# sk4161/EgoScaler

Measured on AMD Instinct MI355X. Metric: clips/sec/GPU (8-frame 224^2, 16-token text) fwd+bwd, higher is better.
Workload: dtype bf16

## Files before the change

egoscaler_amd/_lib.py:

```python
import ctypes
import os

import torch

_HERE = os.path.dirname(os.path.abspath(__file__))
LIB_PATH = os.path.join(_HERE, "lib", "libegomi.so")
_lib = None

c_p = ctypes.c_void_p
c_i = ctypes.c_int
c_d = ctypes.c_double
c_f = ctypes.c_float
c_sz = ctypes.c_size_t
c_i64 = ctypes.c_int64


class EgomiError(RuntimeError):
    pass


def lib():
    global _lib
    if _lib is None:
        if not os.path.exists(LIB_PATH):
            raise EgomiError(f"{LIB_PATH} not found: build it with `python -m egoscaler_amd.build` "
                             "(the product path has no CPU fallback)")
        _lib = ctypes.CDLL(LIB_PATH)
        _lib.egomi_strerror.restype = ctypes.c_char_p
        _lib.egomi_strerror.argtypes = [c_i]
        _lib.egomi_last_launch_error.restype = ctypes.c_char_p
        _lib.egomi_unproject_workspace_bytes.restype = c_sz
        _lib.egomi_unproject_workspace_bytes.argtypes = [c_i] * 4
    return _lib


def check(rc: int, what: str):
    if rc != 0:
        msg = lib().egomi_strerror(rc).decode()
        if rc == -3:
            msg += ": " + lib().egomi_last_launch_error().decode()
        raise EgomiError(f"{what}: egomi error {rc} ({msg})")


_SYNC_DEBUG = os.environ.get("EGOMI_SYNC_DEBUG")


def call(name: str, *args):
    fn = getattr(lib(), name)
    if not _SYNC_DEBUG:
        check(fn(*args), name)
        return
    import traceback
    import torch
    try:
        check(fn(*args), name)
        if not torch.cuda.is_current_stream_capturing():
            torch.cuda.synchronize()
    except BaseException as e:
        with open(_SYNC_DEBUG, "a") as f:
            f.write(f"=== {name} raised {type(e).__name__}: {str(e)[:200]}\n")
            f.write("".join(traceback.format_stack(limit=14)))
            f.write(f"args: {[getattr(a, 'value', a) for a in args]}\n")
        raise
```

egoscaler_amd/csrc/attention.hip:

```cpp
#include "common.h"
#include <math.h>
#include <type_traits>

#define AT_HD 128
__device__ __forceinline__ float fast_exp2(float x) { return __builtin_amdgcn_exp2f(x); }
typedef __attribute__((ext_vector_type(4))) __bf16 bf16x4_t;
typedef __attribute__((address_space(3))) bf16x4_t lds_bf16x4;

struct AttnArgs {
    const bf16_t* q; const bf16_t* k; const bf16_t* v; bf16_t* o; float* lse;
    const bf16_t* dout; float* delta; bf16_t* dq; bf16_t* dk; bf16_t* dv;
    const uint8_t* key_mask;
    int B, H, S;
    long long ld_qkv, ld_o, ld_dqkv;
    float scale;
    int causal;
    const float* rope_cos; const float* rope_sin;
};

__device__ __forceinline__ int sw_off(int row, int ch) {
    return 256 * row + 16 * (ch ^ (((row & 3) << 2) | ((row >> 2) & 3)));
}
__device__ __forceinline__ int rowmap(int reg, int half) {
    return (reg & 3) + 8 * (reg >> 2) + 4 * half;
}
__device__ __forceinline__ uint32_t visible_bits(uint32_t km32, int half, int key0, int qi, int causal) {
    uint32_t t = km32 >> (4 * half);
    if (causal) {
        const int lim = qi - key0 - 4 * half;
        const uint32_t cb = lim < 0 ? 0u : (lim >= 31 ? 0xFFFFFFFFu : ((2u << lim) - 1u));
        t &= cb;
    }
    return t;
}
__device__ __forceinline__ bf16x8 lds_row8(const char* tile, int row, int ch) {
    return *reinterpret_cast<const bf16x8*>(tile + sw_off(row, ch));
}
__device__ __forceinline__ bf16x8 lds_tr8(const char* tile, int r0, int col0, int lane) {
    const int half = lane >> 5, q = (lane >> 2) & 3, p = lane & 3;
    const int col = col0 + 16 * ((lane >> 4) & 1) + 4 * p;
    const int ch = col >> 3, within = (col & 7) * 2;
    const int ra = r0 + 4 * half + q;
    const bf16x4_t lo = __builtin_amdgcn_ds_read_tr16_b64_v4bf16((lds_bf16x4*)(tile + sw_off(ra, ch) + within));
    const bf16x4_t hi = __builtin_amdgcn_ds_read_tr16_b64_v4bf16((lds_bf16x4*)(tile + sw_off(ra + 8, ch) + within));
    bf16x8 r;
    r[0] = lo[0]; r[1] = lo[1]; r[2] = lo[2]; r[3] = lo[3];
    r[4] = hi[0]; r[5] = hi[1]; r[6] = hi[2]; r[7] = hi[3];
    return r;
}
__device__ __forceinline__ bf16x8 pack8(const float* v) {
// ... 1650 lines not shown
            vis &= hi < 0 ? 0u : (hi >= 31 ? 0xFFFFFFFFu : ((2u << hi) - 1u));
#pragma unroll
            for (int r = 0; r < 16; ++r) pv[r] = (vis >> rowmap(r, 0)) & 1u ? pv[r] : 0.f;
        }
#pragma unroll
        for (int g = 0; g < 4; ++g) {
            const f32x4 d4 = *reinterpret_cast<const f32x4*>(sD + 8 * g + 4 * half);
#pragma unroll
            for (int e = 0; e < 4; ++e) ds[4 * g + e] = pv[4 * g + e] * (dp[4 * g + e] - d4[e]);
        }
#pragma unroll
        for (int s2 = 0; s2 < 2; ++s2) {
            const bf16x8 pb = pack8(&pv[8 * s2]);
            const bf16x8 db = pack8(&ds[8 * s2]);
#pragma unroll
            for (int dt = 0; dt < HD / 32; ++dt) {
                dv[dt] = __builtin_amdgcn_mfma_f32_32x32x16_bf16(lds_tr8_t<HD>(sDO, 16 * s2, 32 * dt, lane), pb, dv[dt], 0, 0, 0);
                dk[dt] = __builtin_amdgcn_mfma_f32_32x32x16_bf16(lds_tr8_t<HD>(sQ, 16 * s2, 32 * dt, lane), db, dk[dt], 0, 0, 0);
            }
        }
        asm volatile("s_waitcnt lgkmcnt(0)" ::: "memory");
        __builtin_amdgcn_s_barrier();
    }
    asm volatile("s_waitcnt vmcnt(0)" ::: "memory");
    __builtin_amdgcn_s_barrier();
    store_rows_t<HD>(smem + wave * (HD == 128 ? AT_XBYTES : 32 * 144), dk, a.scale, a.dk + row_base * a.ld_dqkv + h * HD, a.ld_dqkv, kb0 + wave * 32, a.S, lane,
                     a.rope_cos, a.rope_sin);
    store_rows_t<HD>(smem + wave * (HD == 128 ? AT_XBYTES : 32 * 144), dv, 1.0f, a.dv + row_base * a.ld_dqkv + h * HD, a.ld_dqkv, kb0 + wave * 32, a.S, lane);
}

__device__ __forceinline__ void dma4_asm(const void* gbase, uint32_t voff, uint32_t lds_base) {
    asm volatile("s_mov_b32 m0, %2\n\ts_nop 0\n\tglobal_load_lds_dword %0, %1" :: "v"(voff), "s"(gbase), "s"(lds_base) : "memory");
}
template <bool MASKED>
__device__ __forceinline__ void dkdv2_tile(const char* sQ, const char* sDO, const char* sVrows, const float* sL, const float* sD, const bf16x8 (&kf)[8],
                                           f32x16 (&dk)[4], f32x16 (&dv)[4], const float sc2, const uint32_t vis, const int lane, const int half) {
    f32x16 x, dp;
#pragma unroll
    for (int r = 0; r < 16; ++r) { x[r] = 0.f; dp[r] = 0.f; }
    const int row = lane & 31;
    bf16x8 qr[2], dr[2], vr[2];
    qr[0] = lds_row8(sQ, row, half); dr[0] = lds_row8(sDO, row, half); vr[0] = lds_row8(sVrows, row, half);
    __builtin_amdgcn_sched_barrier(0);
#pragma unroll
    for (int ks = 0; ks < 8; ++ks) {
        if (ks + 1 < 8) {
            qr[(ks + 1) & 1] = lds_row8(sQ, row, 2 * (ks + 1) + half);
            dr[(ks + 1) & 1] = lds_row8(sDO, row, 2 * (ks + 1) + half);
            vr[(ks + 1) & 1] = lds_row8(sVrows, row, 2 * (ks + 1) + half);
        }
        x = __builtin_amdgcn_mfma_f32_32x32x16_bf16(qr[ks & 1], kf[ks], x, 0, 0, 0);
        dp = __builtin_amdgcn_mfma_f32_32x32x16_bf16(dr[ks & 1], vr[ks & 1], dp, 0, 0, 0);
    }
    bf16x8 dot[4], qt[4];
#pragma unroll
    for (int dt = 0; dt < 4; ++dt) dot[dt] = lds_tr8(sDO, 0, 32 * dt, lane);
    float pv[16], ds[16];
#pragma unroll
    for (int g = 0; g < 4; ++g) {
        const f32x4 l4 = *reinterpret_cast<const f32x4*>(sL + 8 * g + 4 * half);
#pragma unroll
        for (int e = 0; e < 4; ++e) pv[4 * g + e] = fast_exp2(fmaf(x[4 * g + e], sc2, -l4[e] * 1.4426950408889634f));
    }
    if (MASKED) {
#pragma unroll
        for (int r = 0; r < 16; ++r) pv[r] = (vis >> rowmap(r, 0)) & 1u ? pv[r] : 0.f;
    }
#pragma unroll
    for (int dt = 0; dt < 4; ++dt) qt[dt] = lds_tr8(sQ, 0, 32 * dt, lane);
#pragma unroll
    for (int g = 0; g < 4; ++g) {
        const f32x4 d4 = *reinterpret_cast<const f32x4*>(sD + 8 * g + 4 * half);
#pragma unroll
        for (int e = 0; e < 4; ++e) ds[4 * g + e] = pv[4 * g + e] * (dp[4 * g + e] - d4[e]);
    }
    {
        const bf16x8 pb = pack8(&pv[0]);
        const bf16x8 db = pack8(&ds[0]);
#pragma unroll
        for (int dt = 0; dt < 4; ++dt) dv[dt] = __builtin_amdgcn_mfma_f32_32x32x16_bf16(dot[dt], pb, dv[dt], 0, 0, 0);
#pragma unroll
        for (int dt = 0; dt < 4; ++dt) dot[dt] = lds_tr8(sDO, 16, 32 * dt, lane);
#pragma unroll
        for (int dt = 0; dt < 4; ++dt) dk[dt] = __builtin_amdgcn_mfma_f32_32x32x16_bf16(qt[dt], db, dk[dt], 0, 0, 0);
#pragma unroll
        for (int dt = 0; dt < 4; ++dt) qt[dt] = lds_tr8(sQ, 16, 32 * dt, lane);
    }
    {
        const bf16x8 pb = pack8(&pv[8]);
        const bf16x8 db = pack8(&ds[8]);
#pragma unroll
        for (int dt = 0; dt < 4; ++dt) dv[dt] = __builtin_amdgcn_mfma_f32_32x32x16_bf16(dot[dt], pb, dv[dt], 0, 0, 0);
#pragma unroll
        for (int dt = 0; dt < 4; ++dt) dk[dt] = __builtin_amdgcn_mfma_f32_32x32x16_bf16(qt[dt], db, dk[dt], 0, 0, 0);
    }
}

__global__ __launch_bounds__(256, 2) void attn_bwd_dkdv2_kernel(AttnArgs a) {
    extern __shared__ __attribute__((aligned(16))) char smem[];
    const int lane = threadIdx.x & 63, half = lane >> 5;
    const int wave = __builtin_amdgcn_readfirstlane(threadIdx.x >> 6);
    int rank, h, b;
    attn_block_map(a, rank, h, b);
    const int kb0 = rank * 128;
    const long long row_base = (long long)b * a.S;
    const bf16_t* Q = a.q + row_base * a.ld_qkv + h * AT_HD;
    const bf16_t* K = a.k + row_base * a.ld_qkv + h * AT_HD;
    const bf16_t* V = a.v + row_base * a.ld_qkv + h * AT_HD;
    const bf16_t* DO = a.dout + row_base * a.ld_o + h * AT_HD;
    const float* LSE = a.lse + ((long long)b * a.H + h) * a.S;
    const float* DEL = a.delta + ((long long)b * a.H + h) * a.S;
    const int kj = kb0 + wave * 32 + (lane & 31);
    const int kr = kj < a.S ? kj : a.S - 1;
    bool key_ok = kj < a.S;
    if (key_ok && a.key_mask) key_ok = a.key_mask[row_base + kj] != 0;
    const bool keys_all_ok = __all(key_ok);
    const bool wave_dead = kb0 + wave * 32 >= a.S;
    char* sVblk = smem + 2 * DKV_STAGE;
    const uint32_t lds_smem = (uint32_t)(uintptr_t)((lds_void_t*)smem);
    {
        const uint32_t base = __builtin_amdgcn_readfirstlane(lds_smem + 2 * DKV_STAGE + wave * 8 * 1024);
#pragma unroll
        for (int j = 0; j < 8; ++j) {
            const int rl = (wave * 8 + j) * 4 + (lane >> 4);
            const int ch = (lane & 15) ^ (((rl & 3) << 2) | ((rl >> 2) & 3));
            int r = kb0 + rl;
            r = r < a.S ? r : a.S - 1;
            dma16_asm(V, (uint32_t)((long long)r * a.ld_qkv + ch * 8) * 2u, base + j * 1024);
        }
    }
// ... 20 lines not shown
            const int ch = (lane & 15) ^ (((rl & 3) << 2) | ((rl >> 2) & 3));
            int r = q0 + rl;
            r = r < a.S ? r : a.S - 1;
            qo[j] = (uint32_t)((long long)r * a.ld_qkv + ch * 8) * 2u;
            dofs[j] = (uint32_t)((long long)r * a.ld_o + ch * 8) * 2u;
        }
        int qq = q0 + (lane & 31);
        qq = qq < a.S ? qq : a.S - 1;
        lo = (uint32_t)qq * 4u;
    };
    offsets_for(qt0 * 32, qoff, dooff, loff);
    const uint32_t q_stride = (uint32_t)(32 * a.ld_qkv * 2), do_stride = (uint32_t)(32 * a.ld_o * 2);
    const float* LD = (wave & 1) ? DEL : LSE;
    auto issue = [&](int stage, const uint32_t (&qo)[2], const uint32_t (&dofs)[2], const uint32_t lo) {
        const uint32_t base = __builtin_amdgcn_readfirstlane(lds_smem + stage * DKV_STAGE + wave * 2 * 1024);
#pragma unroll
        for (int j = 0; j < 2; ++j) dma16_asm(Q, qo[j], base + j * 1024);
#pragma unroll
        for (int j = 0; j < 2; ++j) dma16_asm(DO, dofs[j], base + 32 * 256 + j * 1024);
        dma4_asm(LD, lo, __builtin_amdgcn_readfirstlane(lds_smem + stage * DKV_STAGE + 2 * 32 * 256 + wave * 256));
    };
    auto issue_next = [&](int qt_next, int stage) {
        if (ragged && qt_next == nq - 1) {
            uint32_t qo[2], dofs[2], lo;
            offsets_for(qt_next * 32, qo, dofs, lo);
            issue(stage, qo, dofs, lo);
        } else {
            issue(stage, qoff, dooff, loff);
#pragma unroll
            for (int j = 0; j < 2; ++j) { qoff[j] += q_stride; dooff[j] += do_stride; }
            loff += 128u;
        }
    };
    if (qt0 < nq) issue_next(qt0, 0);
    int stg = 0;
    auto top_of_tile = [&](int qt) {
        if (qt + 1 < nq) {
            issue_next(qt + 1, stg ^ 1);
            asm volatile("s_waitcnt vmcnt(5)" ::: "memory");
        } else {
            asm volatile("s_waitcnt vmcnt(0)" ::: "memory");
        }
        asm volatile("s_waitcnt lgkmcnt(0)" ::: "memory");
        __builtin_amdgcn_s_barrier();
    };
    auto end_of_tile = [&]() {
        stg ^= 1;
        asm volatile("s_waitcnt lgkmcnt(0)" ::: "memory");
        __builtin_amdgcn_s_barrier();
    };
    const char* sVrows = sVblk + wave * 32 * 256;
    auto run = [&](auto masked_tag, int qt) {
        constexpr bool MASKED = decltype(masked_tag)::value;
        const char* st = smem + stg * DKV_STAGE;
        const float* sL = reinterpret_cast<const float*>(st + 2 * 32 * 256);
        uint32_t vis = 0u;
        if (MASKED) {
            const int q0 = qt * 32;
            const int lo = a.causal ? kj - q0 - 4 * half : 0;
            const int hi = a.S - 1 - q0 - 4 * half;
            vis = key_ok ? 0xFFFFFFFFu : 0u;
            vis &= lo <= 0 ? 0xFFFFFFFFu : (lo >= 32 ? 0u : ~((1u << lo) - 1u));
            vis &= hi < 0 ? 0u : (hi >= 31 ? 0xFFFFFFFFu : ((2u << hi) - 1u));
        }
        dkdv2_tile<MASKED>(st, st + 32 * 256, sVrows, sL, sL + 64, kf, dk, dv, sc2, vis, lane, half);
    };
    using T_ = std::integral_constant<bool, true>;
    using F_ = std::integral_constant<bool, false>;
    int qt = qt0;
    const int diag = kb0 / 32 + wave;
    const int dead_end = wave_dead ? nq : (a.causal ? (diag < nq ? diag : nq) : qt0);
    for (; qt < dead_end; ++qt) {
        top_of_tile(qt);
        end_of_tile();
    }
    if (a.causal && qt < nq && qt == diag) {
        top_of_tile(qt);
        run(T_{}, qt);
        end_of_tile();
        ++qt;
    }
    if (keys_all_ok) {
        const int int_end = a.S / 32;
        for (; qt < int_end; ++qt) {
            top_of_tile(qt);
            run(F_{}, qt);
            end_of_tile();
        }
    }
    for (; qt < nq; ++qt) {
        top_of_tile(qt);
        run(T_{}, qt);
        end_of_tile();
    }
    store_rows_via_lds(smem + wave * AT_XBYTES, dk, a.scale, a.dk + row_base * a.ld_dqkv + h * AT_HD, a.ld_dqkv, kb0 + wave * 32, a.S, lane,
                       a.rope_cos, a.rope_sin);
    store_rows_via_lds(smem + wave * AT_XBYTES, dv, 1.0f, a.dv + row_base * a.ld_dqkv + h * AT_HD, a.ld_dqkv, kb0 + wave * 32, a.S, lane);
}

static int attn_occ() {
    static int occ = -1;
    if (occ < 0) { const char* e = getenv("EGOMI_ATTN_OCC"); occ = e ? atoi(e) : 3; }
    return occ;
}
static bool occ_dq2() { return attn_occ() & 1; }

static int g_attn_fwd_form = -1;
static int attn_fwd_form() {
    if (g_attn_fwd_form < 0) { const char* e = getenv("EGOMI_ATTN_FWD"); g_attn_fwd_form = e ? atoi(e) : 4; }
    return g_attn_fwd_form;
}
extern "C" int egomi_attn_set_fwd_form(int form) {
    if (form < 1 || form > 4) return EGOMI_E_BADARG;
    g_attn_fwd_form = form;
    return EGOMI_OK;
}
static int g_attn_fwd_group = -1;
static int attn_fwd_group() {
    if (g_attn_fwd_group < 0) { const char* e = getenv("EGOMI_ATTN_GROUP"); g_attn_fwd_group = e ? atoi(e) : 0; }
    return g_attn_fwd_group;
}
extern "C" int egomi_attn_set_fwd_group(int group) {
    if (group < 0 || group > 64) return EGOMI_E_BADARG;
    g_attn_fwd_group = group;
    return EGOMI_OK;
}
static int g_attn_fwd_blocks = 0;
extern "C" int egomi_attn_set_fwd_blocks(int blocks) {
    if (blocks < 0) return EGOMI_E_BADARG;
    g_attn_fwd_blocks = blocks;
    return EGOMI_OK;
}
static int g_attn_bwd_form = -1;
static int attn_bwd_form() {
    if (g_attn_bwd_form < 0) { const char* e = getenv("EGOMI_ATTN_BWD"); g_attn_bwd_form = e ? atoi(e) : 3; }
    return g_attn_bwd_form;
}
extern "C" int egomi_attn_set_bwd_form(int form) {
    if (form < 1 || form > 3) return EGOMI_E_BADARG;
    g_attn_bwd_form = form;
    return EGOMI_OK;
}

static int attn_check(const egomi_attn_desc* d, bool fwd_only = false) {
    if (!d || !d->q || !d->k || !d->v) return EGOMI_E_BADARG;
    if (d->head_dim != AT_HD && d->head_dim != 64) return EGOMI_E_UNSUPPORTED;
    (void)fwd_only;
    if (d->B <= 0 || d->H <= 0 || d->S <= 0) return EGOMI_E_SHAPE;
    if (d->dtype != EGOMI_BF16) return EGOMI_E_UNSUPPORTED;
    if (d->ld_qkv % 8 || d->ld_qkv < d->head_dim * d->H) return EGOMI_E_SHAPE;
    if (((uintptr_t)d->q | (uintptr_t)d->k | (uintptr_t)d->v) & 15) return EGOMI_E_SHAPE;
    return EGOMI_OK;
}

static AttnArgs attn_args(const egomi_attn_desc* d) {
    AttnArgs a;
    a.q = (const bf16_t*)d->q; a.k = (const bf16_t*)d->k; a.v = (const bf16_t*)d->v; a.o = (bf16_t*)d->o; a.lse = d->lse;
    a.dout = (const bf16_t*)d->dout; a.delta = d->delta; a.dq = (bf16_t*)d->dq; a.dk = (bf16_t*)d->dk; a.dv = (bf16_t*)d->dv;
    a.key_mask = d->key_mask; a.B = d->B; a.H = d->H; a.S = d->S;
    a.ld_qkv = d->ld_qkv; a.ld_o = d->ld_o; a.ld_dqkv = d->ld_dqkv; a.scale = d->scale; a.causal = d->causal;
    a.rope_cos = d->rope_cos; a.rope_sin = d->rope_sin;
    return a;
}

extern "C" int egomi_attn_fwd(const egomi_attn_desc* d, egomi_stream_t stream) {
    const int rc = attn_check(d, true);
    if (rc) return rc;
    if (!d->o || d->ld_o % 8 || d->ld_o < d->head_dim * d->H || ((uintptr_t)d->o & 15)) return EGOMI_E_SHAPE;
    if (d->S > AT_MAXS) return EGOMI_E_UNSUPPORTED;
    AttnArgs a = attn_args(d);
    const dim3 grid((unsigned)(((d->S + 127) / 128) * d->H * d->B));
    const size_t lds = 2 * 2 * 64 * 2 * (size_t)d->head_dim + (size_t)((d->S + 63) / 64) * 64;
    int form = attn_fwd_form();
    if ((long long)d->S * d->ld_qkv * 2 >= (1ll << 32)) form = 1;
    if (d->head_dim == 128 && form == 4 && d->S > 1024) form = 3;
    if (d->head_dim == 128 && form == 4) {
        const int s32 = (d->S + 31) & ~31, nblk = (s32 + 127) / 128;
        const int n_items = nblk * d->H * d->B;
        static int cus = 0;
        if (!cus) { int dev = 0; hipDeviceProp_t pr; cus = (hipGetDevice(&dev) == hipSuccess && hipGetDeviceProperties(&pr, dev) == hipSuccess) ? pr.multiProcessorCount : 256; }
        int grid4 = n_items < 2 * cus ? n_items : 2 * cus;
        if (g_attn_fwd_blocks > 0 && g_attn_fwd_blocks < grid4) grid4 = g_attn_fwd_blocks;
        const size_t lds4 = (size_t)F3_NST * F3_STAGE + 4 * F4_STRIP + 2 * (size_t)s32;
        (void)hipFuncSetAttribute(reinterpret_cast<const void*>(attn_fwd4_kernel), hipFuncAttributeMaxDynamicSharedMemorySize, (int)lds4);
        EGOMI_LAUNCH(attn_fwd4_kernel, dim3((unsigned)grid4), dim3(256), lds4, (hipStream_t)stream, a, n_items);
        return egomi_launch_status();
    }
    if (d->head_dim == 128 && form == 3) {
        const int s32 = (d->S + 31) & ~31, nblk = (s32 + 127) / 128;
        int group = (d->H * d->B) % 8 == 0 ? attn_fwd_group() : 0;
        if (group > nblk) group = nblk;
        const int nb = group > 0 ? ((nblk + group - 1) / group) * group : nblk;
        const dim3 grid3((unsigned)(nb * d->H * d->B));
        const size_t lds3 = (size_t)F3_NST * F3_STAGE + (size_t)s32;
        (void)hipFuncSetAttribute(reinterpret_cast<const void*>(attn_fwd3_kernel), hipFuncAttributeMaxDynamicSharedMemorySize, (int)lds3);
        EGOMI_LAUNCH(attn_fwd3_kernel, grid3, dim3(256), lds3, (hipStream_t)stream, a, group);
        return egomi_launch_status();
    }
    if (d->head_dim == 128) {
        if (form == 1) {
            (void)hipFuncSetAttribute(reinterpret_cast<const void*>(attn_fwd_kernel<128>), hipFuncAttributeMaxDynamicSharedMemorySize, (int)lds);
            EGOMI_LAUNCH(attn_fwd_kernel<128>, grid, dim3(256), lds, (hipStream_t)stream, a);
        } else {
            (void)hipFuncSetAttribute(reinterpret_cast<const void*>(attn_fwd2_kernel<128>), hipFuncAttributeMaxDynamicSharedMemorySize, (int)lds);
            EGOMI_LAUNCH(attn_fwd2_kernel<128>, grid, dim3(256), lds, (hipStream_t)stream, a);
        }
    } else if (form == 1) {
        EGOMI_LAUNCH(attn_fwd_kernel<64>, grid, dim3(256), lds, (hipStream_t)stream, a);
    } else {
        EGOMI_LAUNCH(attn_fwd2_kernel<64>, grid, dim3(256), lds, (hipStream_t)stream, a);
    }
    return egomi_launch_status();
}

extern "C" int egomi_attn_bwd(const egomi_attn_desc* d, egomi_stream_t stream) {
    const int rc = attn_check(d);
    if (rc) return rc;
    if (!d->o || !d->lse || !d->dout || !d->delta || !d->dq || !d->dk || !d->dv) return EGOMI_E_BADARG;
    if (d->ld_o % 8 || d->ld_dqkv % 8 || d->ld_o < d->head_dim * d->H || d->ld_dqkv < d->head_dim * d->H) return EGOMI_E_SHAPE;
    if (((uintptr_t)d->dout & 15) || (((uintptr_t)d->dq | (uintptr_t)d->dk | (uintptr_t)d->dv) & 15) || ((uintptr_t)d->o & 15)) return EGOMI_E_SHAPE;
    if (d->S > AT_MAXS) return EGOMI_E_UNSUPPORTED;
    if ((d->rope_cos == nullptr) != (d->rope_sin == nullptr)) return EGOMI_E_BADARG;
    if (d->rope_cos && (((uintptr_t)d->rope_cos | (uintptr_t)d->rope_sin) & 15)) return EGOMI_E_SHAPE;
    AttnArgs a = attn_args(d);
    hipStream_t s = (hipStream_t)stream;
    const dim3 grid((unsigned)(((d->S + 127) / 128) * d->H * d->B));
    if (d->head_dim == 64) {
        if (d->rope_cos) return EGOMI_E_UNSUPPORTED;
        const size_t lq = 2 * 2 * 64 * 128 + (size_t)((d->S + 63) / 64) * 64, lk = 2 * (2 * 32 * 128 + 4 * 256) + 128 * 128;
        EGOMI_LAUNCH((attn_bwd_dq_kernel<2, 64>), grid, dim3(256), lq, s, a);
        EGOMI_LAUNCH((attn_bwd_dkdv_kernel<2, 64>), grid, dim3(256), lk, s, a);
        return egomi_launch_status();
    }
    const size_t lds_q = ((occ_dq2() ? 2 : 3) * 2 * 64 * 256) + (size_t)((d->S + 63) / 64) * 64;
    const int occ = attn_occ();
    const bool off32 = (long long)d->S * d->ld_qkv * 2 < (1ll << 32) && (long long)d->S * d->ld_o * 2 < (1ll << 32);
    if ((occ & 1) && attn_bwd_form() == 3 && off32) {
        const size_t lds3 = (size_t)F3_NST * F3_STAGE + (size_t)((d->S + 31) & ~31);
        (void)hipFuncSetAttribute(reinterpret_cast<const void*>(attn_bwd_dq3_kernel), hipFuncAttributeMaxDynamicSharedMemorySize, (int)lds3);
        EGOMI_LAUNCH(attn_bwd_dq3_kernel, grid, dim3(256), lds3, s, a);
    } else if ((occ & 1) && attn_bwd_form() == 2 && off32) {
        (void)hipFuncSetAttribute(reinterpret_cast<const void*>(attn_bwd_dq2_kernel), hipFuncAttributeMaxDynamicSharedMemorySize, (int)lds_q);
        EGOMI_LAUNCH(attn_bwd_dq2_kernel, grid, dim3(256), lds_q, s, a);
    } else if (occ & 1) {
        (void)hipFuncSetAttribute(reinterpret_cast<const void*>(attn_bwd_dq_kernel<2>), hipFuncAttributeMaxDynamicSharedMemorySize, (int)lds_q);
        EGOMI_LAUNCH(attn_bwd_dq_kernel<2>, grid, dim3(256), lds_q, s, a);
    } else {
        (void)hipFuncSetAttribute(reinterpret_cast<const void*>(attn_bwd_dq_kernel<1>), hipFuncAttributeMaxDynamicSharedMemorySize, (int)lds_q);
        EGOMI_LAUNCH(attn_bwd_dq_kernel<1>, grid, dim3(256), lds_q, s, a);
    }
    const size_t lds_k = (occ & 2) ? 2 * DKV_STAGE + 128 * 256 : 3 * DKV_STAGE;
    if ((occ & 2) && attn_bwd_form() >= 2 && off32) {
        (void)hipFuncSetAttribute(reinterpret_cast<const void*>(attn_bwd_dkdv2_kernel), hipFuncAttributeMaxDynamicSharedMemorySize, (int)lds_k);
        EGOMI_LAUNCH(attn_bwd_dkdv2_kernel, grid, dim3(256), lds_k, s, a);
    } else if (occ & 2) {
        (void)hipFuncSetAttribute(reinterpret_cast<const void*>(attn_bwd_dkdv_kernel<2>), hipFuncAttributeMaxDynamicSharedMemorySize, (int)lds_k);
        EGOMI_LAUNCH(attn_bwd_dkdv_kernel<2>, grid, dim3(256), lds_k, s, a);
    }
    else EGOMI_LAUNCH(attn_bwd_dkdv_kernel<1>, grid, dim3(256), lds_k, s, a);
    return egomi_launch_status();
}
```

egoscaler_amd/engine.py:

```python
import os
from typing import Dict

import torch

from . import ops
from .config import EgoDims


class Workspace:

    def __init__(self, device):
        self.device = device
        self.bufs: Dict[str, torch.Tensor] = {}

    def get(self, name, shape, dtype, zero=False):
        t = self.bufs.get(name)
        shape = tuple(int(s) for s in shape)
        if t is None or t.shape != shape or t.dtype != dtype:
            t = torch.empty(shape, dtype=dtype, device=self.device)
            self.bufs[name] = t
            if zero:
                t.zero_()
        elif zero:
            t.zero_()
# ... 617 lines not shown
            lc = ctx["layers"][l]
            gu, qkv = lc["gu"], lc["qkv"]
            self._begin_direct(l)
            dgu = ws.get("dgu", (M, 2 * Fd), T)
            wt_down = self.wT.get(p + "mlp.down_proj.weight") if self.prepared else None
            if fuse_swiglu_bwd and wt_down is not None and l in self.wguT:
                ops.mm(dx, wt_down, out=dgu, swiglu_bwd_gu=gu)
            else:
                d_act = self._dgrad(dx, p + "mlp.down_proj.weight", ws.get("d_act", (M, Fd), T))
                if self.prepared and l in self.wguT and self.gu_il:
                    ops.swiglu_il_bwd(d_act, gu, dgu)
                else:
                    ops.swiglu_bwd(d_act, gu[:, :Fd], gu[:, Fd:], dgu[:, :Fd], dgu[:, Fd:])
            self._wgrad(p + "mlp.down_proj.weight", dx, lc["act"])
            t_h2 = None
            if self.prepared and l in self.wguT:
                if defer_b:
                    d_h2, t_h2 = ops.mm(dgu, self.wguT[l], out=ws.get("d_h", (M, d), T), defer_tail=True)
                else:
                    d_h2 = ops.mm(dgu, self.wguT[l], out=ws.get("d_h", (M, d), T))
            elif self.prepared and l in self.wgu_cat:
                d_h2 = self._dgrad_w(dgu, self.wgu_cat[l], ws.get("d_h", (M, d), T))
            else:
                d_h2 = self._dgrad(dgu[:, :Fd], p + "mlp.gate_proj.weight", ws.get("d_h", (M, d), T))
                self._dgrad(dgu[:, Fd:], p + "mlp.up_proj.weight", d_h2, residual=d_h2)
            self._wgrad_stacked([p + "mlp.gate_proj.weight", p + "mlp.up_proj.weight"], dgu, lc["h2"])
            n2 = p + "post_attention_layernorm.weight"
            d_mid = ops.rmsnorm_bwd(d_h2, lc["x_mid"], w[n2], lc["rstd2"], dx_add=dx,
                                    dw=self.grad_buffer(n2) if n2 in tr else None, out=ws.get("dx_b", (M, d), T), tail=t_h2)
            d_ao = self._dgrad(d_mid, p + "self_attn.o_proj.weight", ws.get("d_ao", (M, d), T))
            self._wgrad(p + "self_attn.o_proj.weight", d_mid, lc["ao"])
            dqkv = ws.get("dqkv", (M, 3 * d), T)
            if lc["lse"] is not None:
                ops.attn_bwd(qkv, lc["ao"], lc["lse"], d_ao, dqkv, ws.get("att_delta", (B, H, S), torch.float32), B, S, H, hd, scale,
                             causal=True, key_mask=ctx["key_mask"], rope=(self.cos, self.sin))
            else:
                self._attention_bwd(qkv, lc["P"], d_ao, dqkv, B, S, H, hd, scale)
                ops.rope_(dqkv, self.cos, self.sin, M, S, 0, 2 * H, hd, 3 * d, inverse=True)
            t_h = None
            if self.prepared and l in self.wqkvT:
                if defer_b:
                    d_h, t_h = ops.mm(dqkv, self.wqkvT[l], out=ws.get("d_h", (M, d), T), defer_tail=True)
                else:
                    d_h = ops.mm(dqkv, self.wqkvT[l], out=ws.get("d_h", (M, d), T))
            elif self.prepared and l in self.wqkv and self.use_tn and T == torch.bfloat16:
                d_h = self._dgrad_w(dqkv, self.wqkv[l], ws.get("d_h", (M, d), T))
            else:
                d_h = self._dgrad(dqkv[:, :d], p + "self_attn.q_proj.weight", ws.get("d_h", (M, d), T))
                self._dgrad(dqkv[:, d:2 * d], p + "self_attn.k_proj.weight", d_h, residual=d_h)
                self._dgrad(dqkv[:, 2 * d:], p + "self_attn.v_proj.weight", d_h, residual=d_h)
            self._wgrad_stacked([p + f"self_attn.{nm}_proj.weight" for nm in "qkv"], dqkv, lc["h"])
            n1 = p + "input_layernorm.weight"
            dx = ops.rmsnorm_bwd(d_h, lc["x_in"], w[n1], lc["rstd1"], dx_add=d_mid,
                                 dw=self.grad_buffer(n1) if n1 in tr else None, out=ws.get("dx_a", (M, d), T), tail=t_h)
            self._notify_layer(l)
        Pn = pb.point_token_len
        V = lm.vocab_size
        emb_name = "model.embed_tokens.weight"
        Bc = ctx["n_clouds"]
        d_feats = ws.get("d_pp_out", (Bc * Pn, d), T) if ctx["has_points"] else None
        if d_feats is not None:
            d_feats.zero_()
        ops.embed_splice_bwd(dx.view(B, S, d), ctx["ids"], ctx["start_pos"], Pn, V,
                             self.grad_buffer(emb_name) if emb_name in tr else None, d_feats, cloud_idx=ctx["cloud_idx"])
        if ctx["has_points"]:
            acts = ctx["pp_acts"]
            nh = len(pb.projection_hidden_dim)
            g = d_feats
# ... 57 lines not shown
```

egoscaler_amd/ops.py:

```python
import ctypes
import math

import torch

from . import _lib
from ._lib import c_p, c_i, c_d, c_f, c_sz, c_i64, call

F32, BF16 = 0, 1


def dt(t: torch.dtype) -> int:
    if t == torch.float32:
        return F32
    if t == torch.bfloat16:
        return BF16
    raise TypeError(f"unsupported dtype {t}")


def P(t):
    if t is None:
        return c_p(None)
    if not t.is_cuda:
        raise _lib.EgomiError("egoscaler_amd ops need CUDA/HIP tensors (no CPU fallback)")
    return c_p(t.data_ptr())
# ... 475 lines not shown

def add(a, b, out=None):
    out = torch.empty_like(a) if out is None else out
    call("egomi_add", P(a), P(b), P(out), c_i64(a.numel()), c_i(dt(a.dtype)), S())
    return out


def colsum_(x, out):
    R, C = x.shape
    call("egomi_colsum", P(x), c_i64(R), c_i(C), c_i64(_ld(x)), P(out), c_i(dt(x.dtype)), S())
    return out


def group_max(x, BG, M, C, concat=False, out=None):
    if out is None:
        out = torch.empty((BG * M, 2 * C) if concat else (BG, C), dtype=x.dtype, device=x.device)
    call("egomi_group_max", P(x), c_i(BG), c_i(M), c_i(C), P(out), c_i(int(concat)), c_i(dt(x.dtype)), S())
    return out


def linear_smallk(x, w, b, act=0, out=None):
    R, K = x.numel() // x.shape[-1], x.shape[-1]
    N = w.shape[0]
    out = torch.empty(R, N, dtype=w.dtype, device=w.device) if out is None else out
    call("egomi_linear_smallk", P(x), c_i(dt(x.dtype)), P(w), P(b), P(out), c_i64(R), c_i(N), c_i(K), c_i(act), c_i(dt(w.dtype)), S())
    return out


class AttnDesc(ctypes.Structure):
    _fields_ = [("q", c_p), ("k", c_p), ("v", c_p), ("o", c_p), ("lse", c_p),
                ("dout", c_p), ("delta", c_p), ("dq", c_p), ("dk", c_p), ("dv", c_p), ("key_mask", c_p),
                ("B", c_i), ("H", c_i), ("S", c_i), ("head_dim", c_i),
                ("ld_qkv", c_i64), ("ld_o", c_i64), ("ld_dqkv", c_i64),
                ("scale", c_f), ("causal", c_i), ("dtype", c_i), ("rope_cos", c_p), ("rope_sin", c_p)]


def _attn_desc(qkv, B, Sq, H, hd, scale, causal, key_mask):
    d = AttnDesc()
    dm = H * hd
    d.q, d.k, d.v = qkv[:, :dm].data_ptr(), qkv[:, dm:2 * dm].data_ptr(), qkv[:, 2 * dm:].data_ptr()
    d.key_mask = key_mask.data_ptr() if key_mask is not None else None
    d.B, d.H, d.S, d.head_dim = B, H, Sq, hd
    d.ld_qkv = qkv.stride(0)
    d.scale, d.causal, d.dtype = scale, int(causal), dt(qkv.dtype)
    return d


def attn_fwd(qkv, B, Sq, H, hd, scale, out, lse, causal=True, key_mask=None):
    d = _attn_desc(qkv, B, Sq, H, hd, scale, causal, key_mask)
    d.o, d.lse, d.ld_o = out.data_ptr(), lse.data_ptr() if lse is not None else None, out.stride(0)
    call("egomi_attn_fwd", ctypes.byref(d), S())
    return out


def attn_bwd(qkv, out, lse, dout, dqkv, delta, B, Sq, H, hd, scale, causal=True, key_mask=None, rope=None):
    d = _attn_desc(qkv, B, Sq, H, hd, scale, causal, key_mask)
    if rope is not None:
        cos, sin = rope
        if cos.dtype != torch.float32 or sin.dtype != torch.float32 or cos.shape[0] < Sq or cos.shape[1] != hd // 2 \
                or not cos.is_contiguous() or not sin.is_contiguous():
            raise ValueError("attn_bwd: rope tables must be contiguous fp32 [>=S, head_dim/2]")
        d.rope_cos, d.rope_sin = cos.data_ptr(), sin.data_ptr()
    dm = H * hd
    d.o, d.lse, d.ld_o = out.data_ptr(), lse.data_ptr(), out.stride(0)
    if dout.stride(0) != out.stride(0):
        raise ValueError("attn_bwd: dout and out must share their row stride")
    d.dout, d.delta = dout.data_ptr(), delta.data_ptr()
    d.dq, d.dk, d.dv = dqkv[:, :dm].data_ptr(), dqkv[:, dm:2 * dm].data_ptr(), dqkv[:, 2 * dm:].data_ptr()
    d.ld_dqkv = dqkv.stride(0)
    call("egomi_attn_bwd", ctypes.byref(d), S())
    return dqkv
```

include/egomi.h:

```cpp
#ifndef EGOMI_H
#define EGOMI_H
#include <stddef.h>
#include <stdint.h>

#ifdef __cplusplus
extern "C" {
#endif

#define EGOMI_OK 0
#define EGOMI_E_BADARG (-1)
#define EGOMI_E_SHAPE (-2)
#define EGOMI_E_LAUNCH (-3)
#define EGOMI_E_UNSUPPORTED (-4)

#define EGOMI_F32 0
#define EGOMI_BF16 1

typedef void* egomi_stream_t;

int egomi_version(void);
const char* egomi_strerror(int code);
const char* egomi_last_launch_error(void);

size_t egomi_unproject_workspace_bytes(int B, int T, int H, int W);
// ... 25 lines not shown
    float alpha;
    int accumulate;
    int act;
    int force_generic;
    void* workspace; int64_t workspace_bytes; int split_k;
    int ws_tickets_zeroed;
    int epilogue; void* C2; int64_t ldc2;
} egomi_gemm_desc;
#define EGOMI_EPI_NONE 0
#define EGOMI_EPI_SWIGLU 1
#define EGOMI_EPI_SLABS 2
#define EGOMI_EPI_SWIGLU_BWD 3
int egomi_gemm(const egomi_gemm_desc* desc, egomi_stream_t stream);
int egomi_gemm_kernel_id(const egomi_gemm_desc* desc);
int egomi_gemm_set_tall(int mode);
int egomi_gemm_slab_count(const egomi_gemm_desc* desc);
int egomi_gemm_tail_plan(const egomi_gemm_desc* desc, int* row0, int* slices);
int egomi_gemm_tn_tail_plan(const egomi_gemm_desc* desc, int* row0, int* slices);
int egomi_event_create(void** event);
int egomi_event_destroy(void* event);
int egomi_event_elapsed_ms(void* start, void* stop, float* ms);
int egomi_gemm_time_next(void* start, void* stop);

typedef struct egomi_attn_desc {
    const void* q; const void* k; const void* v; void* o; float* lse;
    const void* dout; float* delta; void* dq; void* dk; void* dv;
    const uint8_t* key_mask;
    int B, H, S, head_dim;
    int64_t ld_qkv, ld_o, ld_dqkv;
    float scale;
    int causal;
    int dtype;
    const float* rope_cos; const float* rope_sin;
} egomi_attn_desc;
int egomi_attn_fwd(const egomi_attn_desc* desc, egomi_stream_t stream);
int egomi_attn_bwd(const egomi_attn_desc* desc, egomi_stream_t stream);
int egomi_attn_set_fwd_form(int form);
int egomi_attn_set_fwd_blocks(int blocks);
int egomi_attn_set_fwd_group(int group);
int egomi_attn_set_bwd_form(int form);

int egomi_slabs_rmsnorm(const float* slabs, int slices, int rows, int cols, const void* residual, int64_t ldr, const void* w, float eps,
                        void* x_out, int64_t ldx, void* h_out, int64_t ldh, int dtype, egomi_stream_t stream);
int egomi_qkv_finish(const float* slabs, int slices, void* qkv, int64_t ld, const float* cos_tab, const float* sin_tab, int pos,
                     void* kcache, void* vcache, int B, int H, int hd, int Smax, int dtype, egomi_stream_t stream);
int egomi_kv_append(const void* k, const void* v, int64_t ld, void* kcache, void* vcache, int B, int S, int H, int hd, int Smax,
                    int pos0, int dtype, egomi_stream_t stream);
int egomi_attn_decode(const void* q, int64_t ld_q, const void* kcache, const void* vcache, const uint8_t* key_mask, int64_t ld_mask,
                      void* out, int64_t ld_o, int B, int H, int hd, int Smax, int T_len, float scale, int dtype,
                      egomi_stream_t stream);
int egomi_argmax_rows(const void* logits, int64_t ld, int B, int V, int64_t* ids, int64_t* seq, int64_t ld_seq, int pos, int dtype,
                      egomi_stream_t stream);
int egomi_sample_rows(const void* logits, int64_t ld, int B, int V, float* scores, int64_t ld_scores, int64_t* seq, int64_t ld_seq,
                      int pos, int rep_from, int64_t* ids, int* done, float repetition_penalty, float temperature, int top_k,
                      float top_p, int do_sample, const uint64_t* rng, int draw, int64_t eos_id, int64_t pad_id, int dtype,
                      egomi_stream_t stream);
int egomi_beam_rows(const void* logits, int64_t ld, int lg_div, int R, int V, int nb, float* scores, int64_t ld_scores, const int64_t* seq,
                    int64_t ld_seq, int pos, float repetition_penalty, float temperature, int top_k, float top_p, int min_tokens_to_keep,
                    int do_sample, const uint64_t* rng, int draw, const float* run_score, int K, float* cand_key, float* cand_score,
                    int32_t* cand_tok, const int32_t* ctl, int dtype, egomi_stream_t stream);
int egomi_beam_update(int B, int nb, int K, int V, const float* cand_key, const float* cand_score, const int32_t* cand_tok, int S0, int cur_len,
                      int max_len, int64_t eos_id, float length_penalty, int early_stopping, int64_t* seq, int64_t* fin_seq, int64_t ld_seq,
                      int32_t* beam_idx, int32_t* fin_beam_idx, int64_t ld_bidx, int32_t* kv_row, int64_t ld_kv, float* run_score,
                      float* fin_score, int32_t* fin_flag, int32_t* heur, int64_t* tok, int32_t* ctl, egomi_stream_t stream);
int egomi_attn_decode_rows(const void* q, int64_t ld_q, const void* kcache, const void* vcache, const int32_t* kv_row, int64_t ld_kv,
                           int n_phys, const uint8_t* key_mask, int64_t ld_mask, void* out, int64_t ld_o, int B, int nb, int H, int hd,
                           int Smax, int T_len, float scale, int dtype, egomi_stream_t stream);

int egomi_kv_append_fp8(const void* k, const void* v, int64_t ld, uint8_t* kcodes, uint8_t* vcodes, float* kscale, float* vscale, int B, int S,
// ... 106 lines not shown
```

Baseline: 66.85.

## Materialize dS in dK/dV backward kernel and compute dQ from stored dS

Adds a new default backward form where the dK/dV kernel writes the bf16 dS tiles to a global workspace, and a new dQ kernel reads those tiles plus K to accumulate dQ without recomputing QK^T, softmax and dO·V^T. A separate delta kernel computes rowsum(dO·O) first. The aim is to stop the dQ pass from recomputing the attention probabilities, at the cost of extra global memory traffic and a workspace of B*H*tiles*2KB. The change also adds dummy LDS loads to keep the vmcnt accounting consistent.

```diff
diff --git a/egoscaler_amd/_lib.py b/egoscaler_amd/_lib.py
--- a/egoscaler_amd/_lib.py
+++ b/egoscaler_amd/_lib.py
@@ -31,6 +31,7 @@
         _lib.egomi_last_launch_error.restype = ctypes.c_char_p
         _lib.egomi_unproject_workspace_bytes.restype = c_sz
         _lib.egomi_unproject_workspace_bytes.argtypes = [c_i] * 4
+        _lib.egomi_attn_bwd_ws_bytes.restype = c_sz
     return _lib
 
 
diff --git a/egoscaler_amd/csrc/attention.hip b/egoscaler_amd/csrc/attention.hip
--- a/egoscaler_amd/csrc/attention.hip
+++ b/egoscaler_amd/csrc/attention.hip
@@ -16,6 +16,7 @@
     float scale;
     int causal;
     const float* rope_cos; const float* rope_sin;
+    bf16_t* ds;
 };
 
 __device__ __forceinline__ int sw_off(int row, int ch) {
@@ -1732,9 +1733,16 @@
 __device__ __forceinline__ void dma4_asm(const void* gbase, uint32_t voff, uint32_t lds_base) {
     asm volatile("s_mov_b32 m0, %2\n\ts_nop 0\n\tglobal_load_lds_dword %0, %1" :: "v"(voff), "s"(gbase), "s"(lds_base) : "memory");
 }
-template <bool MASKED>
+__device__ __forceinline__ void ds_store_asm(bf16_t* gtile, const bf16x8 v, int lane) {
+    uint32_t voff;
+    asm volatile("v_mbcnt_lo_u32_b32 %0, -1, 0\n\tv_mbcnt_hi_u32_b32 %0, -1, %0\n\tv_lshlrev_b32 %0, 4, %0\n\tglobal_store_dwordx4 %0, %1, %2"
+                 : "=&v"(voff) : "v"(v), "s"(gtile));
+    (void)lane;
+}
+template <bool MASKED, bool DS = false>
 __device__ __forceinline__ void dkdv2_tile(const char* sQ, const char* sDO, const char* sVrows, const float* sL, const float* sD, const bf16x8 (&kf)[8],
-                                           f32x16 (&dk)[4], f32x16 (&dv)[4], const float sc2, const uint32_t vis, const int lane, const int half) {
+                                           f32x16 (&dk)[4], f32x16 (&dv)[4], const float sc2, const uint32_t vis, const int lane, const int half,
+                                           bf16_t* ds_tile = nullptr) {
     f32x16 x, dp;
 #pragma unroll
     for (int r = 0; r < 16; ++r) { x[r] = 0.f; dp[r] = 0.f; }
@@ -1777,6 +1785,7 @@
     {
         const bf16x8 pb = pack8(&pv[0]);
         const bf16x8 db = pack8(&ds[0]);
+        if (DS) ds_store_asm(ds_tile, db, lane);
 #pragma unroll
         for (int dt = 0; dt < 4; ++dt) dv[dt] = __builtin_amdgcn_mfma_f32_32x32x16_bf16(dot[dt], pb, dv[dt], 0, 0, 0);
 #pragma unroll
@@ -1789,6 +1798,7 @@
     {
         const bf16x8 pb = pack8(&pv[8]);
         const bf16x8 db = pack8(&ds[8]);
+        if (DS) ds_store_asm(ds_tile + 512, db, lane);
 #pragma unroll
         for (int dt = 0; dt < 4; ++dt) dv[dt] = __builtin_amdgcn_mfma_f32_32x32x16_bf16(dot[dt], pb, dv[dt], 0, 0, 0);
 #pragma unroll
@@ -1796,6 +1806,10 @@
     }
 }
 
+__host__ __device__ __forceinline__ int attn_ds_tiles(int nq, int causal) { return causal ? nq * (nq + 1) / 2 : nq * nq; }
+__device__ __forceinline__ int attn_ds_tile(int qt, int kt, int nq, int causal) { return causal ? qt * (qt + 1) / 2 + kt : qt * nq + kt; }
+
+template <bool DS>
 __global__ __launch_bounds__(256, 2) void attn_bwd_dkdv2_kernel(AttnArgs a) {
     extern __shared__ __attribute__((aligned(16))) char smem[];
     const int lane = threadIdx.x & 63, half = lane >> 5;
@@ -1882,12 +1896,22 @@
             loff += 128u;
         }
     };
+    const uint32_t lds_dummy = __builtin_amdgcn_readfirstlane(lds_smem + 2 * DKV_STAGE + 128 * 256 + wave * 256);
+    auto dummy2 = [&]() {
+        if (DS) {
+            uint32_t z;
+            asm volatile("v_mov_b32 %0, 0\n\ts_mov_b32 m0, %2\n\ts_nop 0\n\tglobal_load_lds_dword %0, %1\n\tglobal_load_lds_dword %0, %1"
+                         : "=&v"(z) : "s"(LD), "s"(lds_dummy) : "memory");
+        }
+    };
     if (qt0 < nq) issue_next(qt0, 0);
+    dummy2();
     int stg = 0;
     auto top_of_tile = [&](int qt) {
         if (qt + 1 < nq) {
             issue_next(qt + 1, stg ^ 1);
-            asm volatile("s_waitcnt vmcnt(5)" ::: "memory");
+            if (DS) asm volatile("s_waitcnt vmcnt(7)" ::: "memory");
+            else asm volatile("s_waitcnt vmcnt(5)" ::: "memory");
         } else {
             asm volatile("s_waitcnt vmcnt(0)" ::: "memory");
         }
@@ -1900,6 +1924,8 @@
         __builtin_amdgcn_s_barrier();
     };
     const char* sVrows = sVblk + wave * 32 * 256;
+    const int kt_w = kb0 / 32 + wave;
+    bf16_t* DSP = DS ? a.ds + ((long long)b * a.H + h) * attn_ds_tiles(nq, a.causal) * 1024 : nullptr;
     auto run = [&](auto masked_tag, int qt) {
         constexpr bool MASKED = decltype(masked_tag)::value;
         const char* st = smem + stg * DKV_STAGE;
@@ -1913,7 +1939,12 @@
             vis &= lo <= 0 ? 0xFFFFFFFFu : (lo >= 32 ? 0u : ~((1u << lo) - 1u));
             vis &= hi < 0 ? 0u : (hi >= 31 ? 0xFFFFFFFFu : ((2u << hi) - 1u));
         }
-        dkdv2_tile<MASKED>(st, st + 32 * 256, sVrows, sL, sL + 64, kf, dk, dv, sc2, vis, lane, half);
+        if (DS) {
+            dkdv2_tile<MASKED, true>(st, st + 32 * 256, sVrows, sL, sL + 64, kf, dk, dv, sc2, vis, lane, half,
+                                     DSP + (long long)attn_ds_tile(qt, kt_w, nq, a.causal) * 1024);
+        } else {
+            dkdv2_tile<MASKED>(st, st + 32 * 256, sVrows, sL, sL + 64, kf, dk, dv, sc2, vis, lane, half);
+        }
     };
     using T_ = std::integral_constant<bool, true>;
     using F_ = std::integral_constant<bool, false>;
@@ -1922,6 +1953,7 @@
     const int dead_end = wave_dead ? nq : (a.causal ? (diag < nq ? diag : nq) : qt0);
     for (; qt < dead_end; ++qt) {
         top_of_tile(qt);
+        dummy2();
         end_of_tile();
     }
     if (a.causal && qt < nq && qt == diag) {
@@ -1948,6 +1980,133 @@
     store_rows_via_lds(smem + wave * AT_XBYTES, dv, 1.0f, a.dv + row_base * a.ld_dqkv + h * AT_HD, a.ld_dqkv, kb0 + wave * 32, a.S, lane);
 }
 
+__global__ __launch_bounds__(256) void attn_delta_kernel(const bf16_t* __restrict__ dout, const bf16_t* __restrict__ o, long long ld_o,
+                                                         float* __restrict__ delta, int B, int H, int S) {
+    const long long p = ((long long)blockIdx.x * 256 + threadIdx.x) >> 4;
+    const int lane = threadIdx.x & 63, c = lane & 15;
+    const long long row = p / H;
+    const int h = (int)(p - row * H);
+    const bool ok = row < (long long)B * S;
+    const long long rr = ok ? row : 0;
+    const bf16x8 dv = *reinterpret_cast<const bf16x8*>(dout + rr * ld_o + h * AT_HD + 8 * c);
+    const bf16x8 ov = *reinterpret_cast<const bf16x8*>(o + rr * ld_o + h * AT_HD + 8 * c);
+    float d = 0.f;
+#pragma unroll
+    for (int k = 0; k < 8; ++k) {
+        const float in = __shfl(d, lane >= 2 ? lane - 2 : lane, 64);
+        if ((c >> 1) == k) {
+            d = k ? in : 0.f;
+#pragma unroll
+            for (int e = 0; e < 8; ++e) d = fmaf((float)dv[e], (float)ov[e], d);
+        }
+    }
+    const float other = __shfl(d, lane + 1 < 64 ? lane + 1 : lane, 64);
+    if (ok && c == 14) {
+        const int b = (int)(row / S), sq = (int)(row - (long long)b * S);
+        delta[((long long)b * H + h) * S + sq] = d + other;
+    }
+}
+
+__device__ __forceinline__ bf16x8 ds_frag(const char* tile, int s, int lane) {
+    const int half = lane >> 5, q4 = (lane >> 2) & 3, p = lane & 3;
+    const int key = 16 * s + 4 * half + q4;
+    const int off = 1024 * ((lane >> 4) & 1) + 512 * (p & 1) + 8 * (p >> 1) + 16 * key;
+    const bf16x4_t lo = __builtin_amdgcn_ds_read_tr16_b64_v4bf16((lds_bf16x4*)(tile + off));
+    const bf16x4_t hi = __builtin_amdgcn_ds_read_tr16_b64_v4bf16((lds_bf16x4*)(tile + off + 16 * 8));
+    bf16x8 r;
+    r[0] = lo[0]; r[1] = lo[1]; r[2] = lo[2]; r[3] = lo[3];
+    r[4] = hi[0]; r[5] = hi[1]; r[6] = hi[2]; r[7] = hi[3];
+    return r;
+}
+
+#define DQ4_STAGE (F3_TB + 4 * 2048)
+#define DQ4_NST 3
+__global__ __launch_bounds__(256, 2) void attn_bwd_dq4_kernel(AttnArgs a) {
+    extern __shared__ __attribute__((aligned(16))) char smem[];
+    const int lane = threadIdx.x & 63;
+    const int wave = __builtin_amdgcn_readfirstlane(threadIdx.x >> 6);
+    int rank, h, b;
+    attn_block_map(a, rank, h, b);
+    const int q0 = ((a.S + 31) & ~31) - 128 * (rank + 1);
+    const long long row_base = (long long)b * a.S;
+    const bf16_t* K = a.k + row_base * a.ld_qkv + h * AT_HD;
+    const int wave_q0 = q0 + wave * 32;
+    const int qt_w = wave_q0 < 0 ? -1 : wave_q0 / 32;
+    const int last = q0 + 127 < a.S - 1 ? q0 + 127 : a.S - 1;
+    const int nq = (a.S + F3_KT - 1) / F3_KT;
+    const int ntiles = a.causal ? last / F3_KT + 1 : nq;
+    const bf16_t* DSP = a.ds + ((long long)b * a.H + h) * attn_ds_tiles(nq, a.causal) * 1024;
+    uint32_t koff[2];
+#pragma unroll
+    for (int j = 0; j < 2; ++j) {
+        const int rl = (wave * 2 + j) * 4 + (lane >> 4);
+        const int ch = (lane & 15) ^ (((rl & 3) << 2) | ((rl >> 2) & 3));
+        const int r = rl < a.S ? rl : a.S - 1;
+        koff[j] = (uint32_t)((long long)r * a.ld_qkv + ch * 8) * 2u;
+    }
+    const uint32_t tile_stride = (uint32_t)(F3_KT * a.ld_qkv * 2);
+    const uint32_t lds_smem = (uint32_t)(uintptr_t)((lds_void_t*)smem);
+    auto live = [&](int t) { return qt_w >= 0 && (!a.causal || t <= qt_w); };
+    int next_req = 0;
+    auto request = [&]() {
+        const uint32_t stage = lds_smem + (next_req % DQ4_NST) * DQ4_STAGE;
+        const uint32_t kbase = __builtin_amdgcn_readfirstlane(stage + wave * 2 * 1024);
+        if ((next_req + 1) * F3_KT <= a.S) {
+#pragma unroll
+            for (int j = 0; j < 2; ++j) dma16_asm(K, koff[j], kbase + j * 1024);
+#pragma unroll
+            for (int j = 0; j < 2; ++j) koff[j] += tile_stride;
+        } else {
+#pragma unroll
+            for (int j = 0; j < 2; ++j) {
+                const int rl = (wave * 2 + j) * 4 + (lane >> 4);
+                const int ch = (lane & 15) ^ (((rl & 3) << 2) | ((rl >> 2) & 3));
+                int r = next_req * F3_KT + rl;
+                r = r < a.S ? r : a.S - 1;
+                dma16_asm(K, (uint32_t)((long long)r * a.ld_qkv + ch * 8) * 2u, kbase + j * 1024);
+            }
+        }
+        const int tile = qt_w < 0 ? 0 : attn_ds_tile(qt_w, live(next_req) ? next_req : qt_w, nq, a.causal);
+        const uint32_t dbase = __builtin_amdgcn_readfirstlane(stage + F3_TB + wave * 2048);
+#pragma unroll
+        for (int j = 0; j < 2; ++j) dma16_asm(DSP, (uint32_t)tile * 2048u + j * 1024 + lane * 16, dbase + j * 1024);
+        ++next_req;
+    };
+    request();
+    if (ntiles > 1) request();
+    f32x16 dq[4];
+#pragma unroll
+    for (int dt = 0; dt < 4; ++dt)
+#pragma unroll
+        for (int r = 0; r < 16; ++r) dq[dt][r] = 0.f;
+    for (int t = 0; t < ntiles; ++t) {
+        if (t + 1 < ntiles) asm volatile("s_waitcnt vmcnt(4)" ::: "memory");
+        else asm volatile("s_waitcnt vmcnt(0)" ::: "memory");
+        asm volatile("s_waitcnt lgkmcnt(0)" ::: "memory");
+        __builtin_amdgcn_s_barrier();
+        if (t + 2 < ntiles) request();
+        if (live(t)) {
+            const char* sK = smem + (t % DQ4_NST) * DQ4_STAGE;
+            const char* sD = sK + F3_TB + wave * 2048;
+            bf16x8 kt0[4], kt1[4];
+#pragma unroll
+            for (int dt = 0; dt < 4; ++dt) kt0[dt] = lds_tr8(sK, 0, 32 * dt, lane);
+            const bf16x8 db0 = ds_frag(sD, 0, lane);
+#pragma unroll
+            for (int dt = 0; dt < 4; ++dt) kt1[dt] = lds_tr8(sK, 16, 32 * dt, lane);
+            const bf16x8 db1 = ds_frag(sD, 1, lane);
+#pragma unroll
+            for (int dt = 0; dt < 4; ++dt) dq[dt] = __builtin_amdgcn_mfma_f32_32x32x16_bf16(kt0[dt], db0, dq[dt], 0, 0, 0);
+#pragma unroll
+            for (int dt = 0; dt < 4; ++dt) dq[dt] = __builtin_amdgcn_mfma_f32_32x32x16_bf16(kt1[dt], db1, dq[dt], 0, 0, 0);
+        }
+    }
+    asm volatile("s_waitcnt lgkmcnt(0)" ::: "memory");
+    __builtin_amdgcn_s_barrier();
+    store_rows_via_lds(smem + wave * AT_XBYTES, dq, a.scale, a.dq + row_base * a.ld_dqkv + h * AT_HD, a.ld_dqkv, wave_q0, a.S, lane,
+                       a.rope_cos, a.rope_sin);
+}
+
 static int attn_occ() {
     static int occ = -1;
     if (occ < 0) { const char* e = getenv("EGOMI_ATTN_OCC"); occ = e ? atoi(e) : 3; }
@@ -1983,11 +2142,11 @@
 }
 static int g_attn_bwd_form = -1;
 static int attn_bwd_form() {
-    if (g_attn_bwd_form < 0) { const char* e = getenv("EGOMI_ATTN_BWD"); g_attn_bwd_form = e ? atoi(e) : 3; }
+    if (g_attn_bwd_form < 0) { const char* e = getenv("EGOMI_ATTN_BWD"); g_attn_bwd_form = e ? atoi(e) : 4; }
     return g_attn_bwd_form;
 }
 extern "C" int egomi_attn_set_bwd_form(int form) {
-    if (form < 1 || form > 3) return EGOMI_E_BADARG;
+    if (form < 1 || form > 4) return EGOMI_E_BADARG;
     g_attn_bwd_form = form;
     return EGOMI_OK;
 }
@@ -2010,6 +2169,7 @@
     a.key_mask = d->key_mask; a.B = d->B; a.H = d->H; a.S = d->S;
     a.ld_qkv = d->ld_qkv; a.ld_o = d->ld_o; a.ld_dqkv = d->ld_dqkv; a.scale = d->scale; a.causal = d->causal;
     a.rope_cos = d->rope_cos; a.rope_sin = d->rope_sin;
+    a.ds = (bf16_t*)d->ds_ws;
     return a;
 }
 
@@ -2063,6 +2223,17 @@
     return egomi_launch_status();
 }
 
+#define EGOMI_ATTN_DS_MAX (1ll << 30)
+static long long attn_ds_bytes(const egomi_attn_desc* d) {
+    if (!d || d->head_dim != AT_HD || d->B <= 0 || d->H <= 0 || d->S <= 0 || d->S > AT_MAXS) return 0;
+    if ((long long)d->S * d->ld_qkv * 2 >= (1ll << 32) || (long long)d->S * d->ld_o * 2 >= (1ll << 32)) return 0;
+    const long long n = (long long)d->B * d->H * attn_ds_tiles((d->S + 31) / 32, d->causal) * 2048;
+    return n <= EGOMI_ATTN_DS_MAX ? n : 0;
+}
+extern "C" size_t egomi_attn_bwd_ws_bytes(const egomi_attn_desc* d) {
+    return attn_bwd_form() == 4 && attn_occ() == 3 ? (size_t)attn_ds_bytes(d) : 0;
+}
+
 extern "C" int egomi_attn_bwd(const egomi_attn_desc* d, egomi_stream_t stream) {
     const int rc = attn_check(d);
     if (rc) return rc;
@@ -2085,11 +2256,28 @@
     const size_t lds_q = ((occ_dq2() ? 2 : 3) * 2 * 64 * 256) + (size_t)((d->S + 63) / 64) * 64;
     const int occ = attn_occ();
     const bool off32 = (long long)d->S * d->ld_qkv * 2 < (1ll << 32) && (long long)d->S * d->ld_o * 2 < (1ll << 32);
-    if ((occ & 1) && attn_bwd_form() == 3 && off32) {
+    int form = attn_bwd_form();
+    if (form == 4) {
+        const long long need = (long long)egomi_attn_bwd_ws_bytes(d);
+        if (need > 0 && d->ds_ws && !((uintptr_t)d->ds_ws & 15) && (long long)d->ds_ws_bytes >= need) {
+            const long long n_thr = (long long)d->B * d->S * d->H * 16;
+            EGOMI_LAUNCH(attn_delta_kernel, dim3((unsigned)((n_thr + 255) / 256)), dim3(256), 0, s, (const bf16_t*)d->dout, (const bf16_t*)d->o,
+                         (long long)d->ld_o, d->delta, d->B, d->H, d->S);
+            const size_t lds_k = 2 * DKV_STAGE + 128 * 256 + 4 * 256;
+            (void)hipFuncSetAttribute(reinterpret_cast<const void*>(attn_bwd_dkdv2_kernel<true>), hipFuncAttributeMaxDynamicSharedMemorySize, (int)lds_k);
+            EGOMI_LAUNCH(attn_bwd_dkdv2_kernel<true>, grid, dim3(256), lds_k, s, a);
+            const size_t lds4 = (size_t)DQ4_NST * DQ4_STAGE;
+            (void)hipFuncSetAttribute(reinterpret_cast<const void*>(attn_bwd_dq4_kernel), hipFuncAttributeMaxDynamicSharedMemorySize, (int)lds4);
+            EGOMI_LAUNCH(attn_bwd_dq4_kernel, grid, dim3(256), lds4, s, a);
+            return egomi_launch_status();
+        }
+        form = 3;
+    }
+    if ((occ & 1) && form == 3 && off32) {
         const size_t lds3 = (size_t)F3_NST * F3_STAGE + (size_t)((d->S + 31) & ~31);
         (void)hipFuncSetAttribute(reinterpret_cast<const void*>(attn_bwd_dq3_kernel), hipFuncAttributeMaxDynamicSharedMemorySize, (int)lds3);
         EGOMI_LAUNCH(attn_bwd_dq3_kernel, grid, dim3(256), lds3, s, a);
-    } else if ((occ & 1) && attn_bwd_form() == 2 && off32) {
+    } else if ((occ & 1) && form == 2 && off32) {
         (void)hipFuncSetAttribute(reinterpret_cast<const void*>(attn_bwd_dq2_kernel), hipFuncAttributeMaxDynamicSharedMemorySize, (int)lds_q);
         EGOMI_LAUNCH(attn_bwd_dq2_kernel, grid, dim3(256), lds_q, s, a);
     } else if (occ & 1) {
@@ -2100,9 +2288,9 @@
         EGOMI_LAUNCH(attn_bwd_dq_kernel<1>, grid, dim3(256), lds_q, s, a);
     }
     const size_t lds_k = (occ & 2) ? 2 * DKV_STAGE + 128 * 256 : 3 * DKV_STAGE;
-    if ((occ & 2) && attn_bwd_form() >= 2 && off32) {
-        (void)hipFuncSetAttribute(reinterpret_cast<const void*>(attn_bwd_dkdv2_kernel), hipFuncAttributeMaxDynamicSharedMemorySize, (int)lds_k);
-        EGOMI_LAUNCH(attn_bwd_dkdv2_kernel, grid, dim3(256), lds_k, s, a);
+    if ((occ & 2) && form >= 2 && off32) {
+        (void)hipFuncSetAttribute(reinterpret_cast<const void*>(attn_bwd_dkdv2_kernel<false>), hipFuncAttributeMaxDynamicSharedMemorySize, (int)lds_k);
+        EGOMI_LAUNCH(attn_bwd_dkdv2_kernel<false>, grid, dim3(256), lds_k, s, a);
     } else if (occ & 2) {
         (void)hipFuncSetAttribute(reinterpret_cast<const void*>(attn_bwd_dkdv_kernel<2>), hipFuncAttributeMaxDynamicSharedMemorySize, (int)lds_k);
         EGOMI_LAUNCH(attn_bwd_dkdv_kernel<2>, grid, dim3(256), lds_k, s, a);
diff --git a/egoscaler_amd/engine.py b/egoscaler_amd/engine.py
--- a/egoscaler_amd/engine.py
+++ b/egoscaler_amd/engine.py
@@ -673,8 +673,10 @@
             self._wgrad(p + "self_attn.o_proj.weight", d_mid, lc["ao"])
             dqkv = ws.get("dqkv", (M, 3 * d), T)
             if lc["lse"] is not None:
+                n_ds = ops.attn_bwd_ws_bytes(qkv, B, S, H, hd, causal=True, ld_o=d_ao.stride(0))
                 ops.attn_bwd(qkv, lc["ao"], lc["lse"], d_ao, dqkv, ws.get("att_delta", (B, H, S), torch.float32), B, S, H, hd, scale,
-                             causal=True, key_mask=ctx["key_mask"], rope=(self.cos, self.sin))
+                             causal=True, key_mask=ctx["key_mask"], rope=(self.cos, self.sin),
+                             ds_ws=ws.get("att_ds", (n_ds,), torch.uint8) if n_ds else None)
             else:
                 self._attention_bwd(qkv, lc["P"], d_ao, dqkv, B, S, H, hd, scale)
                 ops.rope_(dqkv, self.cos, self.sin, M, S, 0, 2 * H, hd, 3 * d, inverse=True)
diff --git a/egoscaler_amd/ops.py b/egoscaler_amd/ops.py
--- a/egoscaler_amd/ops.py
+++ b/egoscaler_amd/ops.py
@@ -531,7 +531,8 @@
                 ("dout", c_p), ("delta", c_p), ("dq", c_p), ("dk", c_p), ("dv", c_p), ("key_mask", c_p),
                 ("B", c_i), ("H", c_i), ("S", c_i), ("head_dim", c_i),
                 ("ld_qkv", c_i64), ("ld_o", c_i64), ("ld_dqkv", c_i64),
-                ("scale", c_f), ("causal", c_i), ("dtype", c_i), ("rope_cos", c_p), ("rope_sin", c_p)]
+                ("scale", c_f), ("causal", c_i), ("dtype", c_i), ("rope_cos", c_p), ("rope_sin", c_p),
+                ("ds_ws", c_p), ("ds_ws_bytes", c_sz)]
 
 
 def _attn_desc(qkv, B, Sq, H, hd, scale, causal, key_mask):
@@ -552,7 +553,13 @@
     return out
 
 
-def attn_bwd(qkv, out, lse, dout, dqkv, delta, B, Sq, H, hd, scale, causal=True, key_mask=None, rope=None):
+def attn_bwd_ws_bytes(qkv, B, Sq, H, hd, causal=True, ld_o=None):
+    d = _attn_desc(qkv, B, Sq, H, hd, 1.0, causal, None)
+    d.ld_o = H * hd if ld_o is None else ld_o
+    return int(_lib.lib().egomi_attn_bwd_ws_bytes(ctypes.byref(d)))
+
+
+def attn_bwd(qkv, out, lse, dout, dqkv, delta, B, Sq, H, hd, scale, causal=True, key_mask=None, rope=None, ds_ws=None):
     d = _attn_desc(qkv, B, Sq, H, hd, scale, causal, key_mask)
     if rope is not None:
         cos, sin = rope
@@ -567,5 +574,10 @@
     d.dout, d.delta = dout.data_ptr(), delta.data_ptr()
     d.dq, d.dk, d.dv = dqkv[:, :dm].data_ptr(), dqkv[:, dm:2 * dm].data_ptr(), dqkv[:, 2 * dm:].data_ptr()
     d.ld_dqkv = dqkv.stride(0)
+    need = int(_lib.lib().egomi_attn_bwd_ws_bytes(ctypes.byref(d)))
+    if need > 0:
+        if ds_ws is None or ds_ws.numel() * ds_ws.element_size() < need:
+            ds_ws = torch.empty(need, dtype=torch.uint8, device=dqkv.device)
+        d.ds_ws, d.ds_ws_bytes = ds_ws.data_ptr(), ds_ws.numel() * ds_ws.element_size()
     call("egomi_attn_bwd", ctypes.byref(d), S())
     return dqkv
diff --git a/include/egomi.h b/include/egomi.h
--- a/include/egomi.h
+++ b/include/egomi.h
@@ -81,9 +81,11 @@
     int causal;
     int dtype;
     const float* rope_cos; const float* rope_sin;
+    void* ds_ws; size_t ds_ws_bytes;
 } egomi_attn_desc;
 int egomi_attn_fwd(const egomi_attn_desc* desc, egomi_stream_t stream);
 int egomi_attn_bwd(const egomi_attn_desc* desc, egomi_stream_t stream);
+size_t egomi_attn_bwd_ws_bytes(const egomi_attn_desc* desc);
 int egomi_attn_set_fwd_form(int form);
 int egomi_attn_set_fwd_blocks(int blocks);
 int egomi_attn_set_fwd_group(int group);
```

Measured after the change: 67.11 (median of 6 runs). About the same (+0.4%).
